# Mark-Rindler/PTRT-game-engine

Hardware: AMD Instinct MI355X
Metric: Mrays/s (higher is better)
Workload: dtype f32

## Files before the change

### include/ptrt.h

```cpp
#ifndef PTRT_H
#define PTRT_H

#include <stddef.h>
#include <stdint.h>

#ifdef __cplusplus
extern "C" {
#endif

#define PTRT_ABI_VERSION 6

enum {
    PTRT_OK = 0,
    PTRT_E_INVALID = -1,
    PTRT_E_NO_DEVICE = -2,
    PTRT_E_HIP = -3,
    PTRT_E_NOT_READY = -4,
    PTRT_E_NOMEM = -5
};


typedef struct ptrt_vec3 { float x, y, z; } ptrt_vec3;

typedef struct ptrt_bvh_node {
// ... 214 lines not shown

int ptrt_get_stats(ptrt_ctx *ctx, ptrt_stats *out);

int ptrt_post_frame(ptrt_ctx *ctx, const float *accum, const float *normal, const float *depth,
                    const int32_t *object_id, void *out_rgb8, int out_is_device);

typedef struct ptrt_farm ptrt_farm;
int ptrt_farm_create(ptrt_ctx *const *contexts, int n_contexts, ptrt_farm **out);
int ptrt_farm_bands(const ptrt_farm *farm);
const char *ptrt_farm_transport(const ptrt_farm *farm);
int ptrt_farm_part_is_local(const ptrt_farm *farm, int part);
int ptrt_farm_render(ptrt_farm *farm, int frame_index, int spp, int max_depth, void *out_rgb8, int out_is_device);
int ptrt_farm_gather(ptrt_farm *farm, void *out_rgb8, int out_is_device);
int ptrt_farm_parallel(ptrt_farm *farm, void (*fn)(int part, void *user), void *user);
double ptrt_farm_host_us(const ptrt_farm *farm);
void *ptrt_farm_device_frame(ptrt_farm *farm, void *out_rgb8, int out_is_device);
int ptrt_farm_set_option(ptrt_farm *farm, const char *name, long long value);
int ptrt_farm_sync(ptrt_farm *farm);
void ptrt_farm_destroy(ptrt_farm *farm);

int ptrt_set_option(ptrt_ctx *ctx, const char *name, long long value);
int ptrt_get_option(ptrt_ctx *ctx, const char *name, long long *value);

int ptrt_set_stream(ptrt_ctx *ctx, void *hip_stream);

int ptrt_kernel_ms_history(ptrt_ctx *ctx, float *out_ms, int max_n);

int ptrt_launch_ms_history(ptrt_ctx *ctx, float *trace_ms, float *tail_ms, int max_n);

int ptrt_last_kernel_ms(ptrt_ctx *ctx, float *trace_ms, float *tonemap_ms);


typedef struct ptrt_rt_ctx ptrt_rt_ctx;

typedef struct ptrt_rt_material {
    ptrt_vec3 albedo, specular;
    float metallic, roughness;
    ptrt_vec3 emission;
    float ior, transmission, transmission_roughness, clearcoat, clearcoat_roughness;
    ptrt_vec3 subsurface_color;
    float subsurface_radius, anisotropy, sheen;
    ptrt_vec3 sheen_tint;
    float iridescence, iridescence_thickness;
} ptrt_rt_material;

typedef struct ptrt_rt_mesh {
// ... 33 lines not shown
```

### ptrt-game-engine_amd/csrc/pt_kernels.hip.h

```cpp
#pragma once
#include "pt_device.hip.h"

namespace pt {

struct Camera {
    f3 origin, llc, horizontal, vertical, u, v, w;
    float lens_radius;
};

struct KParams {
    const float4 *mesh_recs;
    const float4 *nodes;
    const float4 *nodes2;
    const int2 *leaves;
    const float4 *tris;
    const int4 *slot_face;
    const float4 *tlas_nodes;
    const int2 *tlas_leaves;
    const int *tlas_mesh_ids;
    const float4 *tlas_heads;
    float inst_c2;
    const float4 *materials;
    const float4 *lights;
    const float2 *blue_noise;
    const float4 *tlas_root_box;
    int tlas_root_ref;
    int n_meshes, n_lights;
    int stack_entries;
    int pair_meshes;
    int pair_tri_slots;
    int pair_max_leaf;
    int tlas_max_leaf;
    int tlas_depth;
    int tlas_any_rounds;
    int pair_split;
    int pm1_full_leaf;
    int pm1_dense;
    int steal;
    int csteal;
    int csteal_min;
    int csteal_follow;
    int csteal_leaf_min;
    int leaf_min;
    int leaf_pairs;
    int fetch_min;
    int n_nodes;
    int top_off;
    int n_tiles;
    int lds_extra;
    int lds_flags;
    int pair_cap;
    int lds_wave, lds_wave_bytes;
    Camera cam;
    f3 sky_top, sky_bottom;
    int use_sky;
    const float4 *env;
    int env_w, env_h;
    int width, height;
    int y0, rows;
    int il_period, il_phase;
// ... 761 lines not shown
```

### ptrt-game-engine_amd/csrc/pt_render.hip.h

```cpp
#pragma once
#include "pt_kernels.hip.h"

namespace pt {

struct CycleAcc;
struct PairLds {
    CycleAcc *cyc;
    int stat_bounce;
    float4 *tris;
    int4 *meshtab;
    float4 *meshbox;
    const float4 *topnodes;
    uint32_t *pairs;
    unsigned long long *best;
    uint32_t *occ;
    uint2 *stack;
    int *leafx;
    uint2 *tstack;
    unsigned long long *lkey;
    unsigned char *owner;
    const float2 *jit;
    const float2 *bn;
    const float4 *lights;
    const float4 *mats;
// ... 80 lines not shown
    p += (size_t)meshes * 32;
    l.topnodes = (const float4 *)p;
    p += (size_t)meshes * TOP_NODES * 64;
    p += (size_t)wave * wave_lds_bytes(meshes, stack_entries);
    l.best = (unsigned long long *)p;
    p += 512;
    l.pairs = (uint32_t *)p;
    p += (size_t)meshes * 128;
    l.occ = (uint32_t *)p;
    p += 256;
    l.stack = (uint2 *)p;
    p += (size_t)stack_entries * 512;
    l.lkey = (unsigned long long *)p;
    p += 512;
    l.owner = (unsigned char *)p;
    l.tris = nullptr;
    l.tstack = nullptr;
    l.leafx = nullptr;
    return l;
}

__device__ unsigned long long g_trav_bounce[64];
__device__ unsigned long long g_trav_rhist[8];
__device__ unsigned long long g_trav_stats[32];
#ifdef PT_MARKS
#define PT_MARK(x) asm volatile("; MARK " x)
#else
#define PT_MARK(x)
#endif
#ifdef PT_TRAV_STATS
struct TravStats {
    unsigned v[8] = {0, 0, 0, 0, 0, 0, 0, 0};
    PT_DEV void wave(int i, int lane) {
        if (lane == __builtin_ctzll(__builtin_amdgcn_ballot_w64(true)))
            ++v[i];
    }
    PT_DEV void lanes(int i) { ++v[i]; }
    PT_DEV void flush(int base, int lane, int bounce = -1) {
        for (int i = 0; i < 8; ++i) {
            unsigned a = v[i];
            for (int off = 32; off > 0; off >>= 1)
                a += __shfl_xor(a, off);
            if (lane == 0 && a) {
                atomicAdd(&g_trav_stats[base + i], (unsigned long long)a);
                if (bounce >= 0)
                    atomicAdd(&g_trav_bounce[(bounce < 3 ? bounce : 3) * 16 + base + i], (unsigned long long)a);
// ... 14 lines not shown
    } while (0)
#define TS_EVENT(slot) atomicAdd(&g_trav_dbg[1025 + (slot)], 1ull)
#define TS_WAVE(i) ts.wave(i, lane)
#define TS_LANE(i) ts.lanes(i)
struct CycleAcc {
    unsigned long long c[8] = {0, 0, 0, 0, 0, 0, 0, 0};
    PT_DEV void flush(int lane) {
        if (lane == 0)
            for (int i = 0; i < 8; ++i)
                atomicAdd(&g_trav_stats[24 + i], c[i]);
    }
};
#define TS_LANES(slot, cond)                                                                                             \
    do {                                                                                                                 \
        const unsigned long long ts_m = __builtin_amdgcn_ballot_w64(cond);                                               \
        if (lane == __builtin_ctzll(__builtin_amdgcn_ballot_w64(true)))                                                   \
            atomicAdd(&g_trav_stats[slot], (unsigned long long)__builtin_popcountll(ts_m));                                 \
    } while (0)
#define TS_RHIST(any, cond)                                                                                              \
    do {                                                                                                                 \
        const int ts_r = __builtin_popcountll(__builtin_amdgcn_ballot_w64(cond));                                        \
        if (lane == __builtin_ctzll(__builtin_amdgcn_ballot_w64(true)))                                                   \
            atomicAdd(&g_trav_rhist[((any) ? 4 : 0) + (ts_r == 0 ? 0 : ts_r <= 16 ? 1 : ts_r <= 32 ? 2 : 3)], 1ull);       \
    } while (0)
#define TS_NOW() __builtin_readcyclecounter()
#define TS_ADD(slot, t) (cyc.c[(slot) - 8] += __builtin_readcyclecounter() - (t))
#define TS_ADDL(slot, t) (L.cyc->c[(slot) - 8] += __builtin_readcyclecounter() - (t))
#ifdef PT_TS_SHADING
constexpr bool TS_SHADING = true;
#else
constexpr bool TS_SHADING = false;
#endif
#define TS_ADDQ(slot, t) do { if (!TS_SHADING) TS_ADD(slot, t); } while (0)
#define TS_ADDLQ(slot, t) do { if (!TS_SHADING) TS_ADDL(slot, t); } while (0)
#else
constexpr bool TS_SHADING = false;
#define TS_ADDQ(slot, t) (void)(t)
#define TS_ADDLQ(slot, t) (void)(t)
struct TravStats {
    PT_DEV void flush(int, int, int = -1) {}
};
#define TS_EVENT(slot)
#define TS_DBG(a, b, c, d)
#define TS_WAVE(i)
#define TS_LANE(i)
struct CycleAcc {
    PT_DEV void flush(int) {}
};
#define TS_LANES(slot, cond)
#define TS_RHIST(any, cond)
#define TS_NOW() 0ull
#define TS_ADD(slot, t) (void)(t)
#define TS_ADDL(slot, t) (void)(t)
#endif

PT_DEV void wave_lds_order() {
    __builtin_amdgcn_wave_barrier();
    asm volatile("" ::: "memory");
}

PT_DEV void wave_sync() { wave_lds_order(); }

PT_DEV int lane_prefix(unsigned long long mask) {
    return __builtin_amdgcn_mbcnt_hi((uint32_t)(mask >> 32), __builtin_amdgcn_mbcnt_lo((uint32_t)mask, 0u));
}

PT_DEV MeshHead staged_mesh_head(const PairLds &L, int i) {
    const float4 a = L.meshbox[2 * i], b = L.meshbox[2 * i + 1];
    MeshHead h;
    h.bmin = mk3(a.x, a.y, a.z);
    h.bmax = mk3(b.x, b.y, b.z);
    h.root_ref = __builtin_amdgcn_readfirstlane(__float_as_int(a.w));
    const int fm = __builtin_amdgcn_readfirstlane(__float_as_int(b.w));
// ... 109 lines not shown
        const unsigned long long bal = __builtin_amdgcn_ballot_w64(hb);
        if (hb) {
            ((uint16_t *)L.pairs)[base + lane_prefix(bal)] = (uint16_t)((uint32_t)lane | ((uint32_t)i << 6));
        }
        base += __builtin_popcountll(bal);
    }
    return base;
}

template <int GEN = 0> PT_DEV void pair_ray_from(const KParams &K, const int4 mt, f3 &o, f3 &d, float &dirScale) {
    dirScale = 1.0f;
    if (mt.z & 1) {
        const float4 *rec = GEN ? (K.tlas_heads + mt.w * TLAS_HEAD_F4) : (K.mesh_recs + mt.w * MESH_REC_F4);
        const f3 lo = xform_point(rec[2], rec[3], rec[4], o);
        const f3 ld = xform_dir(rec[2], rec[3], rec[4], d);
        dirScale = length(ld);
        o = lo;
        d = normalize(ld);
    }
}

PT_DEV bool pm1_full_batch(const KParams &K, int sh) { return K.pm1_full_leaf && (K.pair_max_leaf & ((1 << sh) - 1)) == 0; }

template <bool DENSE = false>
PT_DEV Hit closest_hit_pairs(const KParams &K, const PairLds &L, int lane, bool alive, f3 o, f3 d, int &order) {
    const int P = build_pairs<false, DENSE>(K, L, lane, alive, o, d, T_FAR);
    wave_sync();
    for (int c = 0; c < P; c += 64) {
        const int n = (P - c) < 64 ? (P - c) : 64;
        int sh = 0;
        while (K.pair_split && (n << (sh + 1)) <= 64 && (2 << sh) <= K.pair_max_leaf)
            ++sh;
        const int p = c + (lane >> sh), sub = lane & ((1 << sh) - 1);
        const bool valid = (lane >> sh) < n;
        const uint32_t e = ((const uint16_t *)L.pairs)[valid ? p : 0];
        const int r = (int)(e & 63u), oi = (int)(e >> 6);
        const int4 mt = L.meshtab[oi];
        f3 po = mk3(__shfl(o.x, r), __shfl(o.y, r), __shfl(o.z, r));
        f3 pd = mk3(__shfl(d.x, r), __shfl(d.y, r), __shfl(d.z, r));
        float dirScale;
        pair_ray_from<false>(K, mt, po, pd, dirScale);
        RayO pr;
        pr.o = po;
        pr.d = pd;
        float tb = T_FAR;
        int bi = -1;
        const int iters = (K.pair_max_leaf + (1 << sh) - 1) >> sh;
        if (pm1_full_batch(K, sh)) {
            const float4 *tp = L.tris + (mt.x + sub) * 3 + oi * PAIR_PAD;
            const int step = 3 << sh;
            int bit = -1;
            for (int it = 0; it < iters; ++it, tp += step) {
                const float4 p0 = tp[0], p1 = tp[1], p2 = tp[2];
                asm volatile("" ::"v"(p0.w), "v"(p1.w), "v"(p2.w));
                float t, u, v;
                if (tri_test(mk3(p0.x, p0.y, p0.z), mk3(p1.x, p1.y, p1.z), mk3(p2.x, p2.y, p2.z), pr, tb, t, u, v)) {
                    tb = t;
                    bit = it;
                }
            }
            bi = bit < 0 ? -1 : sub + (bit << sh);
        } else {
            for (int it = 0; it < iters; ++it) {
                const int i = sub + (it << sh);
                const int slot = mt.x + (i < mt.y ? i : 0);
                const float4 *tp = L.tris + slot * 3 + oi * PAIR_PAD;
                const float4 p0 = tp[0], p1 = tp[1], p2 = tp[2];
                asm volatile("" ::"v"(p0.w), "v"(p1.w), "v"(p2.w));
                float t, u, v;
                const bool ok = tri_test(mk3(p0.x, p0.y, p0.z), mk3(p1.x, p1.y, p1.z), mk3(p2.x, p2.y, p2.z), pr, tb, t, u, v);
                if (ok && i < mt.y) {
                    tb = t;
                    bi = i;
                }
            }
        }
        if (valid && bi >= 0) {
            const float tw = (mt.z & 1) ? tb / dirScale : tb;
            const unsigned long long key =
                ((unsigned long long)__float_as_uint(tw) << 32) | ((unsigned long long)(uint32_t)oi << 16) | (uint32_t)bi;
            __hip_atomic_fetch_min(&L.best[r], key, __ATOMIC_RELAXED, __HIP_MEMORY_SCOPE_WORKGROUP);
        }
    }
    wave_sync();
    const unsigned long long key = L.best[lane];
    wave_sync();
    Hit h;
// ... 12 lines not shown
    h.mesh = mt.w;
    h.slot = mt.x + bi;
    h.t_local = h.t;
    if (mt.z & 1) {
        const float4 *rec = K.mesh_recs + mt.w * MESH_REC_F4;
        RayO pr;
        pr.o = xform_point(rec[2], rec[3], rec[4], o);
        pr.d = normalize(xform_dir(rec[2], rec[3], rec[4], d));
        const float4 *tp = L.tris + h.slot * 3 + oi * PAIR_PAD;
        const float4 p0 = tp[0], p1 = tp[1], p2 = tp[2];
        float t, u, v;
        tri_test(mk3(p0.x, p0.y, p0.z), mk3(p1.x, p1.y, p1.z), mk3(p2.x, p2.y, p2.z), pr, T_FAR, t, u, v);
        h.t_local = t;
    }
    return h;
}

template <bool DENSE = false>
PT_DEV bool any_hit_pairs(const KParams &K, const PairLds &L, int lane, bool alive, f3 o, f3 d, float tMax) {
    float *tmaxv = (float *)L.best;
    tmaxv[DENSE ? lane_here(lane) : lane] = tMax;
    const int P = build_pairs<true, DENSE>(K, L, lane, alive, o, d, tMax);
    wave_sync();
    for (int c = 0; c < P; c += 64) {
        const int n = (P - c) < 64 ? (P - c) : 64;
        int sh = 0;
        while ((n << (sh + 1)) <= 64 && (2 << sh) <= K.pair_max_leaf)
            ++sh;
        const int p = c + (lane >> sh), sub = lane & ((1 << sh) - 1);
        const bool valid = (lane >> sh) < n;
        const uint32_t e = ((const uint16_t *)L.pairs)[valid ? p : 0];
        const int r = (int)(e & 63u), oi = (int)(e >> 6);
        const int4 mt = L.meshtab[oi];
        f3 po = mk3(__shfl(o.x, r), __shfl(o.y, r), __shfl(o.z, r));
        f3 pd = mk3(__shfl(d.x, r), __shfl(d.y, r), __shfl(d.z, r));
        float dirScale;
        pair_ray_from<false>(K, mt, po, pd, dirScale);
        RayO pr;
        pr.o = po;
        pr.d = pd;
        float tm = tmaxv[r];
        if (mt.z & 1)
            tm = tm * dirScale;
        bool found = false;
        const int iters = (K.pair_max_leaf + (1 << sh) - 1) >> sh;
        if (pm1_full_batch(K, sh)) {
            const float4 *tp = L.tris + (mt.x + sub) * 3 + oi * PAIR_PAD;
            const int step = 3 << sh;
            for (int it = 0; it < iters; ++it, tp += step) {
                const float4 p0 = tp[0], p1 = tp[1], p2 = tp[2];
                asm volatile("" ::"v"(p0.w), "v"(p1.w), "v"(p2.w));
                float t, u, v;
                found |= tri_test(mk3(p0.x, p0.y, p0.z), mk3(p1.x, p1.y, p1.z), mk3(p2.x, p2.y, p2.z), pr, tm, t, u, v);
            }
        } else {
            for (int it = 0; it < iters; ++it) {
                const int i = sub + (it << sh);
                const int slot = mt.x + (i < mt.y ? i : 0);
                const float4 *tp = L.tris + slot * 3 + oi * PAIR_PAD;
                const float4 p0 = tp[0], p1 = tp[1], p2 = tp[2];
                asm volatile("" ::"v"(p0.w), "v"(p1.w), "v"(p2.w));
                float t, u, v;
                const bool ok = tri_test(mk3(p0.x, p0.y, p0.z), mk3(p1.x, p1.y, p1.z), mk3(p2.x, p2.y, p2.z), pr, tm, t, u, v);
                found |= ok && (i < mt.y);
            }
        }
        if (valid && found)
            L.occ[r] = 1u;
    }
    wave_sync();
    const bool occluded = alive && (L.occ[DENSE ? lane_here(lane) : lane] != 0u);
    wave_sync();
    return occluded;
}

template <int GEN> PT_DEV int4 pair_mesh(const KParams &K, const PairLds &L, int r, int order) {
    if (!GEN)
        return staged_mesh_entry(L, order);
    const int j = GEN == 2 ? order : L.leafx[(order & (TLAS_SLOTS - 1)) * 64 + r] + (order >> 2);
    const int root = __float_as_int(K.tlas_heads[TLAS_HEAD_F4 * j].w), flags = __float_as_int(K.tlas_heads[TLAS_HEAD_F4 * j + 1].w);
// ... 1774 lines not shown
```

### ptrt-game-engine_amd/csrc/ptrt_accel.hip.h

```cpp
#pragma once

namespace {

constexpr int REC_INSTANCE = 1;
constexpr int REC_SHADOW_SKIP = 2;

int rec_flags(const float4 *rec) {
    int flags;
    std::memcpy(&flags, &rec[1].w, 4);
    return flags;
}
void set_rec_flag(float4 *rec, int bit, bool on) {
    const int flags = rec_flags(rec);
    rec[1].w = as_f(on ? flags | bit : flags & ~bit);
}
void set_rec_xform(float4 *rec, const float *inverse, const float *world, const float *normal) {
    for (int r = 0; r < 3; ++r) {
        rec[2 + r] = f4(inverse[r * 4], inverse[r * 4 + 1], inverse[r * 4 + 2], inverse[r * 4 + 3]);
        rec[5 + r] = f4(world[r * 4], world[r * 4 + 1], world[r * 4 + 2], world[r * 4 + 3]);
        rec[8 + r] = f4(normal[r * 4], normal[r * 4 + 1], normal[r * 4 + 2], 0.0f);
    }
}

struct Inv3 {
// ... 733 lines not shown
    if (!R.tris.empty()) {
        const int n = (int)(R.tris.size() / 3);
        hipLaunchKernelGGL(pt::tri_normals_kernel, dim3((n + 255) / 256), dim3(256), 0, c->stream, c->d_tris, n);
        HIP_TRY(c, hipGetLastError());
    }
    if (int rc = upload_tlas(c, mesh_count, tlas_nodes, tlas_node_count, tlas_mesh_indices, tlas_index_count, false))
        return rc;
    c->n_geometry_uploads++;
    c->tlas_refits = 0;
    c->tlas_reorders = 0;
    c->all_single_leaf = S.all_leaf;
    c->any_transform = false;
    for (int m = 0; m < mesh_count; ++m)
        c->any_transform = c->any_transform || meshes[m].has_transform != 0;
    c->stack_entries = R.max_depth < 1 ? 1 : R.max_depth;
    c->pair_tri_slots = (int)(R.tris.size() / 3);
    c->pair_max_leaf = 0;
    for (const int2 &lf : R.leaves)
        if (lf.y > c->pair_max_leaf)
            c->pair_max_leaf = lf.y;
    c->pair_leaf_uniform = c->pair_max_leaf > 0;
    for (const int2 &lf : R.leaves)
        c->pair_leaf_uniform = c->pair_leaf_uniform && lf.y == c->pair_max_leaf;
    if (int rc = upload_instance_pretests(c, meshes, mesh_count))
        return rc;
    c->have_geometry = true;
    return PTRT_OK;
}

int ptrt_update_instances(ptrt_ctx *c, const ptrt_mesh_desc *meshes, int mesh_count, const ptrt_bvh_node *tlas_nodes,
                          int tlas_node_count, const int32_t *tlas_mesh_indices, int tlas_index_count) {
    if (int rc = enter_geometry(c, "ptrt_update_instances",
                                meshes && tlas_nodes && tlas_mesh_indices && tlas_node_count > 0 && tlas_index_count > 0))
        return rc;
    if (mesh_count != c->n_meshes)
        return fail(c, PTRT_E_INVALID, "ptrt_update_instances: %d meshes, %d uploaded (use ptrt_upload_geometry)", mesh_count,
                    c->n_meshes);
    if (int rc = set_device(c))
        return rc;
    if (int rc = upload_tlas(c, mesh_count, tlas_nodes, tlas_node_count, tlas_mesh_indices, tlas_index_count, true))
        return rc;
    HIP_TRY(c, hipStreamSynchronize(c->stream));
    c->any_transform = false;
    c->xf_host_stale = false;
    for (int m = 0; m < mesh_count; ++m) {
        const ptrt_mesh_desc &M = meshes[m];
// ... 328 lines not shown
```

### ptrt-game-engine_amd/csrc/ptrt_capi.hip

```cpp
#include "../../include/ptrt.h"
#include "pt_build.hip.h"
#include "pt_denoise.hip.h"
#include "pt_post.hip.h"
#include "pt_refit.hip.h"
#include "pt_tlas.hip.h"
#include "pt_render.hip.h"
#include "pt_wavefront.hip.h"
#include "pt_async.hip.h"
#include "pt_wireframe.hip.h"
#include "pt_query.hip.h"
#include "rt_render.hip.h"

#include <hip/hip_runtime.h>

#include <cmath>
#include <cstdarg>
#include <cstdio>
#include <climits>
#include <cstring>
#include <map>
#include <mutex>
#include <set>
#include <string>
#include <algorithm>
// ... 69 lines not shown
    bool xf_host_stale = false;
    bool inst_c2_all = false;
    XformStage xf;
    float *d_verts = nullptr;
    int4 *d_slot_face = nullptr;
    int *d_leaf_dst = nullptr;
    int *d_node_dst = nullptr;
    int *d_level_nodes = nullptr;
    std::vector<int> level_offset;
    std::vector<int> mesh_vert_base, mesh_vert_count;
    int n_slots = 0, n_leaves = 0;
    int4 *d_face_src = nullptr;
    int *d_slot_pos = nullptr;
    std::vector<int> mesh_face_base, mesh_face_count, mesh_slot_base, mesh_slot_count;
    std::vector<unsigned char> mesh_rebuildable, mesh_is_soup;
    BuildScratch build;
    std::map<int, hipGraphExec_t> graphs;
    hipStream_t capture_stream = nullptr;
    int use_graphs = 0;
    bool tlas_single_leaf = false, all_single_leaf = false, mats_full = false;
    int stack_entries = 1;
    int pair_meshes = 0, pair_tri_slots = 0, pair_max_leaf = 0;
    bool pair_leaf_uniform = false;
    int tlas_max_leaf = 0, tlas_depth = 0;
    bool have_geometry = false, have_materials = false;

    pt::Camera cam{};
    pt::f3 sky_top{0.6f, 0.7f, 1.0f}, sky_bottom{1.0f, 1.0f, 1.0f};
    int use_sky = 1;
    float4 *d_env = nullptr;
    int env_w = 0, env_h = 0;

    bool dn_on = false, dn_first = true;
    pt::DenoiseSettings dn{};
    float4 *dn_cur4 = nullptr, *dn_c4[2] = {nullptr, nullptr}, *dn_g4[2] = {nullptr, nullptr};
    float4 *dn_h1[2] = {nullptr, nullptr}, *dn_h2[2] = {nullptr, nullptr};
    int *dn_hobj = nullptr;
    float *dn_motion = nullptr, *dn_out = nullptr, *dn_pvp = nullptr;
    int dn_cur = 0;
    int dn_active = 1, mv_active = 1;
    float prev_view_proj[16] = {1, 0, 0, 0, 0, 1, 0, 0, 0, 0, 1, 0, 0, 0, 0, 1};

    int rw = 0, rh = 0;
    float *s_accum = nullptr, *s_normal = nullptr, *s_depth = nullptr;
    int *s_object_id = nullptr;
    int bloom_on = 0;
// ... 7 lines not shown
    int wf_sort = 0;
    uint32_t *wf_st = nullptr, *wf_occ = nullptr, *wf_live = nullptr;
    float *wf_planes = nullptr;
    float4 *wf_hit = nullptr;
    size_t wf_items = 0;
    int wf_trace_blocks = 0;
    size_t wf_trace_lds = 0;
    int n_geometry_uploads = 0, n_instance_updates = 0;
    bool any_transform = false;
    int pair_split = 1;
    int last_mode = 0;
    int async_lanes = 0, shade_min = 32, as_leaf_min = 24;
    uint32_t *as_cursor = nullptr;
    int refill = 1;
    bool refill_eff = false;
    VertexStage verts;
    unsigned int *d_queue = nullptr;
    int sample_sync = -1;
    int sample_sync_eff = 0;
    int pm1_dense_roots = -1;
    int pm1_dense_roots_eff = 0;
    int pm1_full_leaf = -1;
    int pm1_full_leaf_eff = 0;
    int tile_run = 8;
    int ticket_tiles = 1;
    int persist = 0, n_cus = 0;
    int as_blocks[2] = {0, 0};
    size_t as_lds = 0;

    int count_rays = 0, force_geom = -1, force_full = 0, pair_trace = 1, fetch_min = 16, leaf_pairs = 1, steal = 1, leaf_min = 8;
    int atrous_exp = 0;
    int csteal_follow = 1, csteal_leaf_min = 32;
    int csteal = 2, csteal_min = 0;
    int lds_pad = 0;
    int pm1_wg = 1;
    static constexpr int MAX_SPLIT = 4;
    int split = 2, split_eff = 1, pipeline = 1;
    hipStream_t aux_stream[MAX_SPLIT] = {nullptr, nullptr, nullptr, nullptr};
    hipEvent_t split_fork = nullptr, split_join[MAX_SPLIT] = {nullptr, nullptr, nullptr, nullptr};
    bool heads_fresh = false;
    bool touched = true;
    bool escaped = false;
    void *prev_out = nullptr;
    hipStream_t prev_stream = nullptr;
    int prev_split = 0;
    bool pipelined_last = false;
// ... 138 lines not shown
    K.tris = c->d_tris;
    K.slot_face = c->d_slot_face;
    K.tlas_nodes = c->d_tlas_nodes;
    K.tlas_leaves = c->d_tlas_leaves;
    K.tlas_mesh_ids = c->d_tlas_mesh_ids;
    K.tlas_heads = c->d_tlas_heads;
    K.inst_c2 = c->inst_c2;
    K.materials = c->d_materials;
    K.lights = c->d_lights;
    K.blue_noise = c->d_blue;
    K.tlas_root_box = c->d_tlas_root_box;
    K.tlas_root_ref = c->tlas_root_ref;
    K.n_meshes = c->n_meshes;
    K.n_lights = c->n_lights;
    K.stack_entries = c->stack_entries;
    K.pair_meshes = c->pair_meshes;
    K.pair_tri_slots = c->pair_tri_slots;
    K.pair_max_leaf = c->pair_max_leaf;
    K.tlas_max_leaf = c->tlas_max_leaf;
    K.tlas_depth = c->tlas_depth < 1 ? 1 : c->tlas_depth;
    K.tlas_any_rounds = (c->n_meshes > 1024 || c->tlas_rounds) ? 1 : 0;
    K.pair_split = (c->pair_split && !c->any_transform) ? 1 : 0;
    K.pm1_full_leaf = (c->pm1_full_leaf != 0 && c->pair_leaf_uniform) ? 1 : 0;
    K.fetch_min = c->fetch_min > 0 ? c->fetch_min : 64;
    K.pair_cap = merged_pair_cap(c);
    K.n_nodes = c->n_nodes;
    K.leaf_pairs = (c->leaf_pairs && (size_t)c->pair_max_leaf * 64 <= (size_t)pt::LEAF_PAIR_BYTES - 512) ? 1 : 0;
    K.leaf_min = c->leaf_min;
    K.steal = c->steal;
    K.csteal = c->csteal;
    K.csteal_min = c->csteal_min;
    K.csteal_follow = c->csteal_follow;
    K.csteal_leaf_min = c->csteal_leaf_min;
    K.cam = c->cam;
    K.sky_top = c->sky_top;
    K.sky_bottom = c->sky_bottom;
    K.use_sky = c->use_sky;
    K.env = c->d_env;
    K.env_w = c->env_w;
    K.env_h = c->env_h;
    const bool scaled = c->scaled();
    K.width = c->rw;
    K.height = c->rh;
    K.y0 = c->y0;
    K.il_period = c->il_period;
    K.il_phase = c->il_phase;
// ... 630 lines not shown
    const size_t chunks = (n + 63) / 64, slots = (size_t)(c->n_cus > 0 ? c->n_cus : 1) * (size_t)(per_cu > 0 ? per_cu : 1);
    const unsigned grid = (unsigned)(chunks < slots ? chunks : slots);
    hipLaunchKernelGGL((pt::ray_query_kernel<GEOM, PMODE, KIND>), dim3(grid), dim3(64), lds, c->stream, K, o, d, tmax, n, out);
    HIP_TRY(c, hipGetLastError());
    return PTRT_OK;
}
template <int KIND>
int dispatch_query(ptrt_ctx *c, int geom, int pmode, const pt::KParams &K, size_t lds, const float *o, const float *d,
                   const float *tmax, size_t n, void *out) {
    switch (pmode ? pmode : -geom) {
    case 1: return run_query<0, 1, KIND>(c, K, lds, o, d, tmax, n, out);
    case 2: return run_query<1, 2, KIND>(c, K, lds, o, d, tmax, n, out);
    case 3: return run_query<2, 3, KIND>(c, K, lds, o, d, tmax, n, out);
    case 0: return run_query<0, 0, KIND>(c, K, lds, o, d, tmax, n, out);
    case -1: return run_query<1, 0, KIND>(c, K, lds, o, d, tmax, n, out);
    default: return run_query<2, 0, KIND>(c, K, lds, o, d, tmax, n, out);
    }
}
int launch_query(ptrt_ctx *c, int kind, const float *o, const float *d, const float *tmax, size_t n, void *out) {
    const pt::KParams K = make_params(c);
    const int geom = pick_geom(c);
    const int pmode = pair_mode(c, geom, false);
    c->query_pmode = pmode;
    const size_t lds = trace_lds_bytes(c, geom, pmode);
    if (pmode == 3)
        if (int rc = refresh_tlas_heads(c, false))
            return rc;
    return kind == PTRT_QUERY_CLOSEST ? dispatch_query<pt::QUERY_CLOSEST>(c, geom, pmode, K, lds, o, d, tmax, n, out)
                                      : dispatch_query<pt::QUERY_OCCLUDED>(c, geom, pmode, K, lds, o, d, tmax, n, out);
}

bool device_span(ptrt_ctx *c, const void *p, size_t bytes) {
    hipPointerAttribute_t a{};
    if (hipPointerGetAttributes(&a, p) != hipSuccess) {
        (void)hipGetLastError();
        return false;
    }
    if (a.type != hipMemoryTypeDevice || a.device != c->device)
        return false;
    hipDeviceptr_t base = nullptr;
    size_t size = 0;
    if (hipMemGetAddressRange(&base, &size, (hipDeviceptr_t)p) != hipSuccess) {
        (void)hipGetLastError();
        return false;
    }
    const size_t off = (size_t)((const char *)p - (const char *)base);
// ... 437 lines not shown
```

### ptrt-game-engine_amd/csrc/ptrt_host_capi.cpp

```cpp
#include "../host/ptrt/scene.hpp"
#include "../host/ptrt/serialize.hpp"
#include "../host/ptrt/farm.hpp"
#include "../host/ptrt/view.hpp"

#include <chrono>
#include <cstring>
#include <string>

namespace {
thread_local std::string g_err;

Material from_floats(const float *m) {
    Material r;
    r.albedo = vec3(m[0], m[1], m[2]);
    r.specular = vec3(m[3], m[4], m[5]);
    r.metallic = m[6];
    r.roughness = m[7];
    r.emission = vec3(m[8], m[9], m[10]);
    r.ior = m[11];
    r.transmission = m[12];
    r.transmissionRoughness = m[13];
    r.clearcoat = m[14];
    r.clearcoatRoughness = m[15];
    r.subsurfaceColor = vec3(m[16], m[17], m[18]);
    r.subsurfaceRadius = m[19];
    r.anisotropy = m[20];
// ... 14 lines not shown
    m[19] = r.subsurfaceRadius; m[20] = r.anisotropy; m[21] = r.sheen;
    m[22] = r.sheenTint.x; m[23] = r.sheenTint.y; m[24] = r.sheenTint.z;
    m[25] = r.iridescence; m[26] = r.iridescenceThickness;
}
int mesh_index(Scene *s, Mesh *m) {
    for (size_t i = 0; i < s->getMeshCount(); ++i)
        if (s->getMesh(i) == m)
            return (int)i;
    return -1;
}
}

#define HS_TRY(body)                                                                                            \
    try {                                                                                                       \
        body;                                                                                                   \
    } catch (const std::exception &e) {                                                                         \
        g_err = e.what();                                                                                       \
        return -1;                                                                                              \
    }

extern "C" {

const char *hs_last_error(void) { return g_err.c_str(); }

void hs_material_default(float *out27) { to_floats(Material(), out27); }
void hs_material_make(const float *albedo3, float roughness, float metallic, float *out27) {
    to_floats(Material(vec3(albedo3[0], albedo3[1], albedo3[2]), roughness, metallic), out27);
}

void *hs_scene_create(int w, int h, int tile_y0, int tile_rows, int device) {
    try {
        return new Scene(w, h, tile_y0, tile_rows, device);
    } catch (const std::exception &e) {
        g_err = e.what();
        return nullptr;
    }
}
void *hs_scene_create_interleaved(int w, int h, int phase, int period, int device) {
    try {
        return new Scene(w, h, Scene::Interleave{phase, period}, device);
    } catch (const std::exception &e) {
        g_err = e.what();
        return nullptr;
    }
}
int hs_tile_rows(void *s) { return static_cast<Scene *>(s)->getTileRows(); }
// ... 384 lines not shown
```

### ptrt-game-engine_amd/csrc/ptrt_options.hip.h

```cpp
#pragma once

namespace {

template <class Launch> int run_check(ptrt_ctx *c, unsigned int *out9, Launch launch) {
    if (int rc = set_device(c))
        return rc;
    DeviceTemp<unsigned int> d;
    HIP_TRY(c, d.alloc(9));
    HIP_TRY(c, hipMemset(d.p, 0, 9 * sizeof(unsigned int)));
    launch(d.p);
    HIP_TRY(c, hipStreamSynchronize(c->stream));
    HIP_TRY(c, hipMemcpy(out9, d.p, 9 * sizeof(unsigned int), hipMemcpyDeviceToHost));
    return PTRT_OK;
}

enum OptPolicy {
    OPT_READ_ONLY,
    OPT_BOOL,
    OPT_REJECT,
    OPT_CLAMP,
    OPT_MASK,
    OPT_TRISTATE,
    OPT_SNAP_124,
};
// ... 10 lines not shown
const Option OPTIONS[] = {
    {"count_rays", &ptrt_ctx::count_rays, OPT_BOOL},
    {"force_geom", &ptrt_ctx::force_geom, OPT_REJECT, -1, 2},
    {"force_full", &ptrt_ctx::force_full, OPT_BOOL},
    {"pair_trace", &ptrt_ctx::pair_trace, OPT_BOOL},
    {"steal", &ptrt_ctx::steal, OPT_REJECT, 0, 64},
    {"csteal", &ptrt_ctx::csteal, OPT_REJECT, 0, 64},
    {"atrous_exp", &ptrt_ctx::atrous_exp, OPT_BOOL},
    {"csteal_follow", &ptrt_ctx::csteal_follow, OPT_BOOL},
    {"csteal_leaf_min", &ptrt_ctx::csteal_leaf_min, OPT_REJECT, 1, 64},
    {"csteal_min", &ptrt_ctx::csteal_min, OPT_REJECT, 0, 1024},
    {"lds_nodes", &ptrt_ctx::lds_nodes, OPT_CLAMP, 0, 2},
    {"merged", &ptrt_ctx::merged, OPT_TRISTATE},
    {"leaf_pairs", &ptrt_ctx::leaf_pairs, OPT_BOOL},
    {"lds_pad", &ptrt_ctx::lds_pad, OPT_REJECT, 0, 32768},
    {"time_kernels", &ptrt_ctx::time_kernels, OPT_BOOL},
    {"time_launches", &ptrt_ctx::time_launches, OPT_BOOL},
    {"tm_prio", &ptrt_ctx::tm_prio, OPT_MASK, 0, 3},
    {"pipeline", &ptrt_ctx::pipeline, OPT_BOOL},
    {"persist", &ptrt_ctx::persist, OPT_CLAMP, 0, INT_MAX},
    {"sample_sync", &ptrt_ctx::sample_sync, OPT_TRISTATE},
    {"pm1_dense_roots", &ptrt_ctx::pm1_dense_roots, OPT_TRISTATE},
    {"pm1_full_leaf", &ptrt_ctx::pm1_full_leaf, OPT_TRISTATE},
    {"tile_run", &ptrt_ctx::tile_run, OPT_REJECT, 0, 64},
    {"ticket_tiles", &ptrt_ctx::ticket_tiles, OPT_CLAMP, 1, 16},
    {"refill", &ptrt_ctx::refill, OPT_CLAMP, 0, 2},
    {"split", &ptrt_ctx::split, OPT_REJECT, 1, ptrt_ctx::MAX_SPLIT},
    {"tlas_rounds", &ptrt_ctx::tlas_rounds, OPT_BOOL},
    {"pm1_wg", &ptrt_ctx::pm1_wg, OPT_REJECT, 0, 2},
    {"stage", &ptrt_ctx::stage, OPT_MASK, 0, 7},
    {"pair_split", &ptrt_ctx::pair_split, OPT_BOOL},
    {"async_lanes", &ptrt_ctx::async_lanes, OPT_BOOL},
    {"shade_min", &ptrt_ctx::shade_min, OPT_REJECT, 1, 64},
    {"leaf_min", &ptrt_ctx::leaf_min, OPT_REJECT, 1, 64, nullptr, [](ptrt_ctx *c, int v) { c->leaf_min = c->as_leaf_min = v; }},
    {"wavefront", &ptrt_ctx::wavefront, OPT_BOOL},
    {"wf_sort", &ptrt_ctx::wf_sort, OPT_SNAP_124},
    {"fetch_min", &ptrt_ctx::fetch_min, OPT_REJECT, 0, 64},
    {"denoiser_active", &ptrt_ctx::dn_active, OPT_BOOL},
    {"motion_vectors", &ptrt_ctx::mv_active, OPT_BOOL},
    {"use_graphs", &ptrt_ctx::use_graphs, OPT_BOOL},
    {"sample_sync_eff", &ptrt_ctx::sample_sync_eff, OPT_READ_ONLY},
    {"pm1_dense_roots_eff", &ptrt_ctx::pm1_dense_roots_eff, OPT_READ_ONLY},
    {"pm1_full_leaf_eff", &ptrt_ctx::pm1_full_leaf_eff, OPT_READ_ONLY},
    {"refilled", nullptr, OPT_READ_ONLY, 0, 0, [](const ptrt_ctx *c) -> long long { return c->refill_eff ? 1 : 0; }},
    {"split_eff", &ptrt_ctx::split_eff, OPT_READ_ONLY},
    {"pipelined", nullptr, OPT_READ_ONLY, 0, 0, [](const ptrt_ctx *c) -> long long { return c->pipelined_last ? 1 : 0; }},
    {"render_mode", &ptrt_ctx::last_mode, OPT_READ_ONLY},
    {"pmode", &ptrt_ctx::last_pmode, OPT_READ_ONLY},
    {"merged_eff", &ptrt_ctx::merged_eff, OPT_READ_ONLY},
    {"merged_decided", nullptr, OPT_READ_ONLY, 0, 0,
     [](const ptrt_ctx *c) -> long long { return (c->merged >= 0 || c->tune_choice >= 0 || !c->last_merged_possible) ? 1 : 0; }},
    {"launches", nullptr, OPT_READ_ONLY, 0, 0, [](const ptrt_ctx *c) { return (long long)c->launches; }},
    {"query_pmode", &ptrt_ctx::query_pmode, OPT_READ_ONLY},
    {"inst_pre_ok", nullptr, OPT_READ_ONLY, 0, 0, [](const ptrt_ctx *c) -> long long { return c->inst_pre_ok ? 1 : 0; }},
    {"tlas_refits", &ptrt_ctx::tlas_refits, OPT_READ_ONLY},
    {"tlas_reorders", &ptrt_ctx::tlas_reorders, OPT_READ_ONLY},
    {"stream", nullptr, OPT_READ_ONLY, 0, 0, [](const ptrt_ctx *c) { return (long long)(intptr_t)c->stream; }},
};

const Option *find_option(const char *name) {
    for (const Option &o : OPTIONS)
        if (std::strcmp(o.name, name) == 0)
            return &o;
    return nullptr;
}

// ... 54 lines not shown
int ptrt_debug_trav_bounce(ptrt_ctx *c, unsigned long long *out64) {
    if (!ctx_live(c) || !out64)
        return fail(c, PTRT_E_INVALID, "ptrt_debug_trav_bounce: bad argument");
    if (int rc = set_device(c))
        return rc;
    HIP_TRY(c, hipStreamSynchronize(c->stream));
    HIP_TRY(c, hipMemcpyFromSymbol(out64, HIP_SYMBOL(pt::g_trav_bounce), 64 * sizeof(unsigned long long)));
    unsigned long long zero[64] = {};
    HIP_TRY(c, hipMemcpyToSymbol(HIP_SYMBOL(pt::g_trav_bounce), zero, sizeof(zero)));
    return PTRT_OK;
}

#ifdef PT_TRAV_STATS
int ptrt_debug_trav_rhist(ptrt_ctx *c, unsigned long long *out8) {
    if (!ctx_live(c) || !out8)
        return fail(c, PTRT_E_INVALID, "ptrt_debug_trav_rhist: bad argument");
    HIP_TRY(c, hipStreamSynchronize(c->stream));
    HIP_TRY(c, hipMemcpyFromSymbol(out8, HIP_SYMBOL(pt::g_trav_rhist), 8 * sizeof(unsigned long long)));
    unsigned long long zero[8] = {};
    HIP_TRY(c, hipMemcpyToSymbol(HIP_SYMBOL(pt::g_trav_rhist), zero, sizeof(zero)));
    return PTRT_OK;
}

int ptrt_debug_trav_dbg(ptrt_ctx *c, unsigned long long *out1033) {
    if (!ctx_live(c) || !out1033)
        return fail(c, PTRT_E_INVALID, "ptrt_debug_trav_dbg: bad argument");
    HIP_TRY(c, hipStreamSynchronize(c->stream));
    HIP_TRY(c, hipMemcpyFromSymbol(out1033, HIP_SYMBOL(pt::g_trav_dbg), 1033 * sizeof(unsigned long long)));
    static unsigned long long zero[1033] = {};
    HIP_TRY(c, hipMemcpyToSymbol(HIP_SYMBOL(pt::g_trav_dbg), zero, sizeof(zero)));
    return PTRT_OK;
}
#endif

int ptrt_debug_rcp_check(ptrt_ctx *c, unsigned int *out9) {
    if (!ctx_live(c) || !out9)
        return fail(c, PTRT_E_INVALID, "ptrt_debug_rcp_check: bad argument");
    return run_check(c, out9, [c](unsigned int *d) { hipLaunchKernelGGL(pt::rcp_check_kernel, dim3(4096), dim3(256), 0, c->stream, d); });
}

int ptrt_debug_rcp_above_check(ptrt_ctx *c, unsigned int *out9) {
    if (!ctx_live(c) || !out9)
        return fail(c, PTRT_E_INVALID, "ptrt_debug_rcp_above_check: bad argument");
    return run_check(c, out9, [c](unsigned int *d) { hipLaunchKernelGGL(pt::rcp_above_check_kernel, dim3(4096), dim3(256), 0, c->stream, d); });
}

// ... 54 lines not shown
```

### ptrt-game-engine_amd/csrc/ptrt_render.hip.h

```cpp
#pragma once

namespace {

int pick_geom(ptrt_ctx *c) {
    int g = c->tlas_single_leaf ? (c->all_single_leaf ? 0 : 1) : 2;
    if (c->force_geom > g)
        g = c->force_geom;
    return g;
}

int merged_pair_cap(const ptrt_ctx *c) {
    const size_t rest = (size_t)c->pair_meshes * 32 + 512 + 256 + (size_t)c->stack_entries * 64 * sizeof(uint2) + pt::LEAF_PAIR_BYTES + 24;
    const int lo = 64 * c->pair_meshes + 64, hi = 128 * c->pair_meshes;
    int cap = rest < 10240 ? (int)((10240 - rest) / 2) / 64 * 64 : 0;
    cap = cap < lo ? lo : cap;
    return cap > hi ? hi : cap;
}

size_t pair_lds_bytes(const ptrt_ctx *c, int pmode) {
    if (pmode == 4)
        return (size_t)c->pair_meshes * 32 + 512 + 256 + (size_t)merged_pair_cap(c) * 2 +
               (size_t)c->stack_entries * 64 * sizeof(uint2) + pt::LEAF_PAIR_BYTES + 24;
    if (pmode == 3)
        return ((size_t)c->tlas_max_leaf * 64 + pt::TLAS_FILL_TARGET) * 2 + 512 * pt::TLAS_SLOTS +
// ... 421 lines not shown
        WAVEFRONT,
        ASYNC,
    } shape = TILES;
    int geom = 0, pmode = 0, pm1_wg = 1;
    bool full = false, tuning = false;
    int tiles_y = 0, grid = 0;
    size_t lds = 0;
    bool one_launch_only() const { return shape != TILES; }
};

int plan_frame(ptrt_ctx *c, pt::KParams &K, int spp, int max_depth, FramePlan &P) {
    K.sample_sync = c->sample_sync >= 0 ? c->sample_sync : (max_depth <= 4 ? 1 : 0);
    c->sample_sync_eff = K.sample_sync;
    P.tiles_y = (K.rows + 7) / 8;
    P.grid = K.tiles_x * P.tiles_y;
    P.geom = pick_geom(c);
    P.full = c->mats_full || c->force_full;
    P.tuning = choose_loop_shape(c, spp, max_depth, P.geom);
    const int pmode = P.pmode = pair_mode(c, P.geom, c->merged_eff != 0);
    c->last_pmode = pmode;
    K.pm1_dense = (pmode == 1 && (c->pm1_dense_roots >= 0 ? c->pm1_dense_roots : (c->pair_meshes >= 4 ? 1 : 0))) ? 1 : 0;
    c->pm1_dense_roots_eff = K.pm1_dense;
    c->pm1_full_leaf_eff = pmode == 1 ? K.pm1_full_leaf : 0;
    if (c->merged < 0 && pmode == 4 && c->csteal == 0)
        K.steal = 0;
    const size_t lds = trace_lds_bytes(c, P.geom, pmode);
    const size_t lds_main = pmode == 1 ? pm1_layout(c, K, P.full, P.grid, P.pm1_wg) : lds + (size_t)c->lds_pad;
    if (c->launches == 0 && getenv("PTRT_DEBUG_LDS"))
        fprintf(stderr, "ptrt: pmode %d, %d meshes in the leaf, %d triangle slots, stack %d, LDS %zu + %zu bytes per workgroup\n", pmode,
                c->pair_meshes, c->pair_tri_slots, c->stack_entries, lds, lds_main - lds);
    P.shape = async_applicable(c)                                 ? FramePlan::ASYNC
              : wavefront_applicable(c, spp, max_depth)           ? FramePlan::WAVEFRONT
              : pmode == 1 && P.pm1_wg == 2                       ? FramePlan::PM1_WG2
              : pmode == 2 && c->lds_nodes && c->stack_entries > 0 ? FramePlan::LDS_NODES
                                                                  : FramePlan::TILES;
    switch (P.shape) {
    case FramePlan::ASYNC: P.lds = async_lds_bytes(c); break;
    case FramePlan::WAVEFRONT: P.lds = wavefront_lds_bytes(c); break;
    case FramePlan::PM1_WG2: P.lds = lds_main; break;
    case FramePlan::LDS_NODES: P.lds = lds_nodes_bytes(c); break;
    case FramePlan::TILES: P.lds = pmode ? lds_main : lds; break;
    }
    if (P.shape == FramePlan::LDS_NODES && P.lds > 64 * 1024)
        return fail(c, PTRT_E_INVALID, "lds_nodes: %zu bytes of LDS per workgroup", P.lds);
    return PTRT_OK;
}
// ... 340 lines not shown
```

Measured before the change: 28560.

## Plan non-power-of-two lane groups for pair leaf triangle batches

Adds a host-built cost-model plan that picks, for each pending pair count, a lane group size that divides the leaf triangle count, not only powers of two, along with how many pairs to take per batch. The kernel reads the plan from kernel params and uses a multiply-shift division to map lanes to pairs and sub-slots. This aims to cut idle lanes and iterations when leaf sizes such as 3 or 6 do not fit power-of-two splits. It grows KParams by 512 bytes and adds per-lane integer multiplies, plus debug counters that compile out by default.

```diff
diff --git a/include/ptrt.h b/include/ptrt.h
--- a/include/ptrt.h
+++ b/include/ptrt.h
@@ -260,6 +260,10 @@
 int ptrt_set_option(ptrt_ctx *ctx, const char *name, long long value);
 int ptrt_get_option(ptrt_ctx *ctx, const char *name, long long *value);
 
+int ptrt_pm1_plan(int leaf_triangles, int32_t *out_g63, int32_t *out_take63, int32_t *out_mul63, int32_t *out_cost63,
+                  int32_t *out_model2);
+int ptrt_pm1_div_mul(int g);
+
 int ptrt_set_stream(ptrt_ctx *ctx, void *hip_stream);
 
 int ptrt_kernel_ms_history(ptrt_ctx *ctx, float *out_ms, int max_n);
diff --git a/ptrt-game-engine_amd/csrc/pm1_plan.h b/ptrt-game-engine_amd/csrc/pm1_plan.h
--- /dev/null
+++ b/ptrt-game-engine_amd/csrc/pm1_plan.h
@@ -0,0 +1,67 @@
+#pragma once
+#include <cstdint>
+
+namespace pt {
+
+constexpr int PM1_BODY = 45, PM1_HEADER = 54;
+constexpr int PM1_MAX_LEAF = 255;
+constexpr int PM1_DIV_SHIFT = 12;
+
+struct Pm1Entry {
+    uint32_t w;
+    uint32_t m;
+};
+struct Pm1Plan {
+    Pm1Entry e[64];
+};
+
+inline uint32_t pm1_div_mul(int g) { return (uint32_t)((1 << PM1_DIV_SHIFT) / g + 1); }
+inline bool pm1_div_exact(int g) {
+    if (g < 1)
+        return false;
+    for (int lane = 0; lane < 64; ++lane)
+        if ((int)(((uint32_t)lane * pm1_div_mul(g)) >> PM1_DIV_SHIFT) != lane / g)
+            return false;
+    return true;
+}
+
+inline int pm1_present_shift(int L, int n, int *iters = nullptr) {
+    int sh = 0;
+    while ((n << (sh + 1)) <= 64 && (2 << sh) <= L)
+        ++sh;
+    if (iters)
+        *iters = (L + (1 << sh) - 1) >> sh;
+    return sh;
+}
+
+inline bool pm1_build_plan(int L, Pm1Plan *plan, int *cost64 = nullptr) {
+    int cost[64], count[64];
+    cost[0] = count[0] = 0;
+    plan->e[0] = Pm1Entry{0u, 0u};
+    const bool ok = L >= 1 && L <= PM1_MAX_LEAF;
+    for (int n = 1; n < 64; ++n) {
+        plan->e[n] = Pm1Entry{(uint32_t)n << 8, 0u};
+        int it;
+        pm1_present_shift(ok ? L : 1, n, &it);
+        cost[n] = it * PM1_BODY + PM1_HEADER;
+        count[n] = 1;
+        for (int g = 1; ok && g <= L && g <= 64; ++g) {
+            if (L % g || !pm1_div_exact(g))
+                continue;
+            const int cap = 64 / g, take = n < cap ? n : cap;
+            const int cst = (L / g) * PM1_BODY + PM1_HEADER + cost[n - take], cnt = 1 + count[n - take];
+            const bool present = (plan->e[n].w & 0xffu) == 0;
+            if (cst < cost[n] || (cst == cost[n] && (cnt < count[n] || (cnt == count[n] && present)))) {
+                cost[n] = cst;
+                count[n] = cnt;
+                plan->e[n] = Pm1Entry{(uint32_t)g | (uint32_t)take << 8 | (uint32_t)(L / g) << 16, pm1_div_mul(g)};
+            }
+        }
+    }
+    if (cost64)
+        for (int n = 0; n < 64; ++n)
+            cost64[n] = cost[n];
+    return ok;
+}
+
+}
diff --git a/ptrt-game-engine_amd/csrc/pt_kernels.hip.h b/ptrt-game-engine_amd/csrc/pt_kernels.hip.h
--- a/ptrt-game-engine_amd/csrc/pt_kernels.hip.h
+++ b/ptrt-game-engine_amd/csrc/pt_kernels.hip.h
@@ -1,5 +1,6 @@
 #pragma once
 #include "pt_device.hip.h"
+#include "pm1_plan.h"
 
 namespace pt {
 
@@ -36,6 +37,8 @@
     int pair_split;
     int pm1_full_leaf;
     int pm1_dense;
+    int pm1_groups;
+    Pm1Plan pm1_plan;
     int steal;
     int csteal;
     int csteal_min;
diff --git a/ptrt-game-engine_amd/csrc/pt_render.hip.h b/ptrt-game-engine_amd/csrc/pt_render.hip.h
--- a/ptrt-game-engine_amd/csrc/pt_render.hip.h
+++ b/ptrt-game-engine_amd/csrc/pt_render.hip.h
@@ -126,6 +126,7 @@
 
 __device__ unsigned long long g_trav_bounce[64];
 __device__ unsigned long long g_trav_rhist[8];
+__device__ unsigned long long g_trav_pm1[2 * 68];
 __device__ unsigned long long g_trav_stats[32];
 #ifdef PT_MARKS
 #define PT_MARK(x) asm volatile("; MARK " x)
@@ -186,6 +187,20 @@
         const int ts_r = __builtin_popcountll(__builtin_amdgcn_ballot_w64(cond));                                        \
         if (lane == __builtin_ctzll(__builtin_amdgcn_ballot_w64(true)))                                                   \
             atomicAdd(&g_trav_rhist[((any) ? 4 : 0) + (ts_r == 0 ? 0 : ts_r <= 16 ? 1 : ts_r <= 32 ? 2 : 3)], 1ull);       \
+    } while (0)
+#define TS_PM1_CALL(any, P)                                                                                              \
+    do {                                                                                                                 \
+        if (lane == __builtin_ctzll(__builtin_amdgcn_ballot_w64(true))) {                                                 \
+            atomicAdd(&g_trav_pm1[((any) ? 68 : 0) + 2], 1ull);                                                          \
+            atomicAdd(&g_trav_pm1[((any) ? 68 : 0) + ((P) > 0 ? 4 + ((P) & 63) : 3)], 1ull);                             \
+        }                                                                                                                \
+    } while (0)
+#define TS_PM1_BATCH(any, iters)                                                                                         \
+    do {                                                                                                                 \
+        if (lane == __builtin_ctzll(__builtin_amdgcn_ballot_w64(true))) {                                                 \
+            atomicAdd(&g_trav_pm1[((any) ? 68 : 0)], (unsigned long long)(iters));                                       \
+            atomicAdd(&g_trav_pm1[((any) ? 68 : 0) + 1], 1ull);                                                          \
+        }                                                                                                                \
     } while (0)
 #define TS_NOW() __builtin_readcyclecounter()
 #define TS_ADD(slot, t) (cyc.c[(slot) - 8] += __builtin_readcyclecounter() - (t))
@@ -213,6 +228,8 @@
 };
 #define TS_LANES(slot, cond)
 #define TS_RHIST(any, cond)
+#define TS_PM1_CALL(any, P)
+#define TS_PM1_BATCH(any, iters)
 #define TS_NOW() 0ull
 #define TS_ADD(slot, t) (void)(t)
 #define TS_ADDL(slot, t) (void)(t)
@@ -368,17 +385,44 @@
 
 PT_DEV bool pm1_full_batch(const KParams &K, int sh) { return K.pm1_full_leaf && (K.pair_max_leaf & ((1 << sh) - 1)) == 0; }
 
+struct PairBatch {
+    int g, take, iters, q, sub;
+    bool full;
+};
+PT_DEV PairBatch pair_batch(const KParams &K, int lane, int n, bool split) {
+    PairBatch B;
+    const Pm1Entry e = (K.pm1_groups && split) ? K.pm1_plan.e[n & 63] : Pm1Entry{0u, 0u};
+    if (e.w & 0xffu) {
+        B.g = (int)(e.w & 0xffu);
+        B.take = (int)((e.w >> 8) & 0xffu);
+        B.iters = (int)(e.w >> 16);
+        B.q = (int)(((uint32_t)lane * e.m) >> PM1_DIV_SHIFT);
+        B.sub = lane - B.q * B.g;
+        B.full = true;
+        return B;
+    }
+    int sh = 0;
+    while (split && (n << (sh + 1)) <= 64 && (2 << sh) <= K.pair_max_leaf)
+        ++sh;
+    B.g = 1 << sh;
+    B.take = n;
+    B.iters = (K.pair_max_leaf + (1 << sh) - 1) >> sh;
+    B.q = lane >> sh;
+    B.sub = lane & ((1 << sh) - 1);
+    B.full = pm1_full_batch(K, sh);
+    return B;
+}
+
 template <bool DENSE = false>
 PT_DEV Hit closest_hit_pairs(const KParams &K, const PairLds &L, int lane, bool alive, f3 o, f3 d, int &order) {
     const int P = build_pairs<false, DENSE>(K, L, lane, alive, o, d, T_FAR);
     wave_sync();
-    for (int c = 0; c < P; c += 64) {
+    TS_PM1_CALL(false, P);
+    for (int c = 0, take = 64; c < P; c += take) {
         const int n = (P - c) < 64 ? (P - c) : 64;
-        int sh = 0;
-        while (K.pair_split && (n << (sh + 1)) <= 64 && (2 << sh) <= K.pair_max_leaf)
-            ++sh;
-        const int p = c + (lane >> sh), sub = lane & ((1 << sh) - 1);
-        const bool valid = (lane >> sh) < n;
+        const PairBatch B = pair_batch(K, lane, n, K.pair_split != 0);
+        const int p = c + B.q, sub = B.sub;
+        const bool valid = B.q < B.take;
         const uint32_t e = ((const uint16_t *)L.pairs)[valid ? p : 0];
         const int r = (int)(e & 63u), oi = (int)(e >> 6);
         const int4 mt = L.meshtab[oi];
@@ -391,10 +435,12 @@
         pr.d = pd;
         float tb = T_FAR;
         int bi = -1;
-        const int iters = (K.pair_max_leaf + (1 << sh) - 1) >> sh;
-        if (pm1_full_batch(K, sh)) {
+        const int iters = B.iters;
+        take = B.take;
+        TS_PM1_BATCH(false, iters);
+        if (B.full) {
             const float4 *tp = L.tris + (mt.x + sub) * 3 + oi * PAIR_PAD;
-            const int step = 3 << sh;
+            const int step = 3 * B.g;
             int bit = -1;
             for (int it = 0; it < iters; ++it, tp += step) {
                 const float4 p0 = tp[0], p1 = tp[1], p2 = tp[2];
@@ -405,10 +451,10 @@
                     bit = it;
                 }
             }
-            bi = bit < 0 ? -1 : sub + (bit << sh);
+            bi = bit < 0 ? -1 : sub + bit * B.g;
         } else {
             for (int it = 0; it < iters; ++it) {
-                const int i = sub + (it << sh);
+                const int i = sub + it * B.g;
                 const int slot = mt.x + (i < mt.y ? i : 0);
                 const float4 *tp = L.tris + slot * 3 + oi * PAIR_PAD;
                 const float4 p0 = tp[0], p1 = tp[1], p2 = tp[2];
@@ -467,13 +513,12 @@
     tmaxv[DENSE ? lane_here(lane) : lane] = tMax;
     const int P = build_pairs<true, DENSE>(K, L, lane, alive, o, d, tMax);
     wave_sync();
-    for (int c = 0; c < P; c += 64) {
+    TS_PM1_CALL(true, P);
+    for (int c = 0, take = 64; c < P; c += take) {
         const int n = (P - c) < 64 ? (P - c) : 64;
-        int sh = 0;
-        while ((n << (sh + 1)) <= 64 && (2 << sh) <= K.pair_max_leaf)
-            ++sh;
-        const int p = c + (lane >> sh), sub = lane & ((1 << sh) - 1);
-        const bool valid = (lane >> sh) < n;
+        const PairBatch B = pair_batch(K, lane, n, true);
+        const int p = c + B.q, sub = B.sub;
+        const bool valid = B.q < B.take;
         const uint32_t e = ((const uint16_t *)L.pairs)[valid ? p : 0];
         const int r = (int)(e & 63u), oi = (int)(e >> 6);
         const int4 mt = L.meshtab[oi];
@@ -488,10 +533,12 @@
         if (mt.z & 1)
             tm = tm * dirScale;
         bool found = false;
-        const int iters = (K.pair_max_leaf + (1 << sh) - 1) >> sh;
-        if (pm1_full_batch(K, sh)) {
+        const int iters = B.iters;
+        take = B.take;
+        TS_PM1_BATCH(true, iters);
+        if (B.full) {
             const float4 *tp = L.tris + (mt.x + sub) * 3 + oi * PAIR_PAD;
-            const int step = 3 << sh;
+            const int step = 3 * B.g;
             for (int it = 0; it < iters; ++it, tp += step) {
                 const float4 p0 = tp[0], p1 = tp[1], p2 = tp[2];
                 asm volatile("" ::"v"(p0.w), "v"(p1.w), "v"(p2.w));
@@ -500,7 +547,7 @@
             }
         } else {
             for (int it = 0; it < iters; ++it) {
-                const int i = sub + (it << sh);
+                const int i = sub + it * B.g;
                 const int slot = mt.x + (i < mt.y ? i : 0);
                 const float4 *tp = L.tris + slot * 3 + oi * PAIR_PAD;
                 const float4 p0 = tp[0], p1 = tp[1], p2 = tp[2];
diff --git a/ptrt-game-engine_amd/csrc/ptrt_accel.hip.h b/ptrt-game-engine_amd/csrc/ptrt_accel.hip.h
--- a/ptrt-game-engine_amd/csrc/ptrt_accel.hip.h
+++ b/ptrt-game-engine_amd/csrc/ptrt_accel.hip.h
@@ -779,6 +779,7 @@
     c->pair_leaf_uniform = c->pair_max_leaf > 0;
     for (const int2 &lf : R.leaves)
         c->pair_leaf_uniform = c->pair_leaf_uniform && lf.y == c->pair_max_leaf;
+    c->pm1_plan_ok = c->pair_leaf_uniform && pt::pm1_build_plan(c->pair_max_leaf, &c->pm1_plan);
     if (int rc = upload_instance_pretests(c, meshes, mesh_count))
         return rc;
     c->have_geometry = true;
diff --git a/ptrt-game-engine_amd/csrc/ptrt_capi.hip b/ptrt-game-engine_amd/csrc/ptrt_capi.hip
--- a/ptrt-game-engine_amd/csrc/ptrt_capi.hip
+++ b/ptrt-game-engine_amd/csrc/ptrt_capi.hip
@@ -115,6 +115,8 @@
     int stack_entries = 1;
     int pair_meshes = 0, pair_tri_slots = 0, pair_max_leaf = 0;
     bool pair_leaf_uniform = false;
+    pt::Pm1Plan pm1_plan{};
+    bool pm1_plan_ok = false;
     int tlas_max_leaf = 0, tlas_depth = 0;
     bool have_geometry = false, have_materials = false;
 
@@ -168,6 +170,8 @@
     int pm1_dense_roots_eff = 0;
     int pm1_full_leaf = -1;
     int pm1_full_leaf_eff = 0;
+    int pm1_lane_groups = -1;
+    int pm1_lane_groups_eff = 0;
     int tile_run = 8;
     int ticket_tiles = 1;
     int persist = 0, n_cus = 0;
@@ -352,6 +356,9 @@
     K.tlas_any_rounds = (c->n_meshes > 1024 || c->tlas_rounds) ? 1 : 0;
     K.pair_split = (c->pair_split && !c->any_transform) ? 1 : 0;
     K.pm1_full_leaf = (c->pm1_full_leaf != 0 && c->pair_leaf_uniform) ? 1 : 0;
+    K.pm1_groups = (c->pm1_lane_groups != 0 && K.pm1_full_leaf && c->pm1_plan_ok) ? 1 : 0;
+    if (K.pm1_groups)
+        K.pm1_plan = c->pm1_plan;
     K.fetch_min = c->fetch_min > 0 ? c->fetch_min : 64;
     K.pair_cap = merged_pair_cap(c);
     K.n_nodes = c->n_nodes;
@@ -1028,6 +1035,7 @@
     const int geom = pick_geom(c);
     const int pmode = pair_mode(c, geom, false);
     c->query_pmode = pmode;
+    c->pm1_lane_groups_eff = pmode == 1 ? K.pm1_groups : 0;
     const size_t lds = trace_lds_bytes(c, geom, pmode);
     if (pmode == 3)
         if (int rc = refresh_tlas_heads(c, false))
diff --git a/ptrt-game-engine_amd/csrc/ptrt_host_capi.cpp b/ptrt-game-engine_amd/csrc/ptrt_host_capi.cpp
--- a/ptrt-game-engine_amd/csrc/ptrt_host_capi.cpp
+++ b/ptrt-game-engine_amd/csrc/ptrt_host_capi.cpp
@@ -2,6 +2,7 @@
 #include "../host/ptrt/serialize.hpp"
 #include "../host/ptrt/farm.hpp"
 #include "../host/ptrt/view.hpp"
+#include "pm1_plan.h"
 
 #include <chrono>
 #include <cstring>
@@ -62,6 +63,29 @@
 extern "C" {
 
 const char *hs_last_error(void) { return g_err.c_str(); }
+
+int ptrt_pm1_plan(int leaf_triangles, int32_t *out_g63, int32_t *out_take63, int32_t *out_mul63, int32_t *out_cost63,
+                  int32_t *out_model2) {
+    if (leaf_triangles < 1 || !out_g63 || !out_take63)
+        return -1;
+    pt::Pm1Plan plan;
+    int cost[64];
+    const bool ok = pt::pm1_build_plan(leaf_triangles, &plan, cost);
+    for (int n = 1; n < 64; ++n) {
+        out_g63[n - 1] = (int32_t)(plan.e[n].w & 0xffu);
+        out_take63[n - 1] = (int32_t)((plan.e[n].w >> 8) & 0xffu);
+        if (out_mul63)
+            out_mul63[n - 1] = (int32_t)plan.e[n].m;
+        if (out_cost63)
+            out_cost63[n - 1] = cost[n];
+    }
+    if (out_model2) {
+        out_model2[0] = pt::PM1_BODY;
+        out_model2[1] = pt::PM1_HEADER;
+    }
+    return ok ? 1 : 0;
+}
+int ptrt_pm1_div_mul(int g) { return (g >= 1 && g <= 64 && pt::pm1_div_exact(g)) ? (int)pt::pm1_div_mul(g) : 0; }
 
 void hs_material_default(float *out27) { to_floats(Material(), out27); }
 void hs_material_make(const float *albedo3, float roughness, float metallic, float *out27) {
diff --git a/ptrt-game-engine_amd/csrc/ptrt_options.hip.h b/ptrt-game-engine_amd/csrc/ptrt_options.hip.h
--- a/ptrt-game-engine_amd/csrc/ptrt_options.hip.h
+++ b/ptrt-game-engine_amd/csrc/ptrt_options.hip.h
@@ -56,6 +56,7 @@
     {"sample_sync", &ptrt_ctx::sample_sync, OPT_TRISTATE},
     {"pm1_dense_roots", &ptrt_ctx::pm1_dense_roots, OPT_TRISTATE},
     {"pm1_full_leaf", &ptrt_ctx::pm1_full_leaf, OPT_TRISTATE},
+    {"pm1_lane_groups", &ptrt_ctx::pm1_lane_groups, OPT_TRISTATE},
     {"tile_run", &ptrt_ctx::tile_run, OPT_REJECT, 0, 64},
     {"ticket_tiles", &ptrt_ctx::ticket_tiles, OPT_CLAMP, 1, 16},
     {"refill", &ptrt_ctx::refill, OPT_CLAMP, 0, 2},
@@ -76,6 +77,7 @@
     {"sample_sync_eff", &ptrt_ctx::sample_sync_eff, OPT_READ_ONLY},
     {"pm1_dense_roots_eff", &ptrt_ctx::pm1_dense_roots_eff, OPT_READ_ONLY},
     {"pm1_full_leaf_eff", &ptrt_ctx::pm1_full_leaf_eff, OPT_READ_ONLY},
+    {"pm1_lane_groups_eff", &ptrt_ctx::pm1_lane_groups_eff, OPT_READ_ONLY},
     {"refilled", nullptr, OPT_READ_ONLY, 0, 0, [](const ptrt_ctx *c) -> long long { return c->refill_eff ? 1 : 0; }},
     {"split_eff", &ptrt_ctx::split_eff, OPT_READ_ONLY},
     {"pipelined", nullptr, OPT_READ_ONLY, 0, 0, [](const ptrt_ctx *c) -> long long { return c->pipelined_last ? 1 : 0; }},
@@ -176,6 +178,16 @@
     return PTRT_OK;
 }
 
+int ptrt_debug_trav_pm1(ptrt_ctx *c, unsigned long long *out136) {
+    if (!ctx_live(c) || !out136)
+        return fail(c, PTRT_E_INVALID, "ptrt_debug_trav_pm1: bad argument");
+    HIP_TRY(c, hipStreamSynchronize(c->stream));
+    HIP_TRY(c, hipMemcpyFromSymbol(out136, HIP_SYMBOL(pt::g_trav_pm1), 136 * sizeof(unsigned long long)));
+    unsigned long long zero[136] = {};
+    HIP_TRY(c, hipMemcpyToSymbol(HIP_SYMBOL(pt::g_trav_pm1), zero, sizeof(zero)));
+    return PTRT_OK;
+}
+
 int ptrt_debug_trav_dbg(ptrt_ctx *c, unsigned long long *out1033) {
     if (!ctx_live(c) || !out1033)
         return fail(c, PTRT_E_INVALID, "ptrt_debug_trav_dbg: bad argument");
diff --git a/ptrt-game-engine_amd/csrc/ptrt_render.hip.h b/ptrt-game-engine_amd/csrc/ptrt_render.hip.h
--- a/ptrt-game-engine_amd/csrc/ptrt_render.hip.h
+++ b/ptrt-game-engine_amd/csrc/ptrt_render.hip.h
@@ -467,6 +467,7 @@
     K.pm1_dense = (pmode == 1 && (c->pm1_dense_roots >= 0 ? c->pm1_dense_roots : (c->pair_meshes >= 4 ? 1 : 0))) ? 1 : 0;
     c->pm1_dense_roots_eff = K.pm1_dense;
     c->pm1_full_leaf_eff = pmode == 1 ? K.pm1_full_leaf : 0;
+    c->pm1_lane_groups_eff = pmode == 1 ? K.pm1_groups : 0;
     if (c->merged < 0 && pmode == 4 && c->csteal == 0)
         K.steal = 0;
     const size_t lds = trace_lds_bytes(c, P.geom, pmode);
```

After: 29280 (median of 6 runs). 1.03x the previous value.
